# hangxu0304/DeepReduce

Measured on NVIDIA H100. Metric: ResNet-50 images/sec (whole job, device-timed, max over ranks), higher is better.
Workload: dtype bf16

## Files before the change

deepreduce_b200/ops/csrc/bn.cu:

```cuda
#include <cuda_bf16.h>

#include <algorithm>

#include "common.cuh"
#include "ops.h"

namespace dr {

namespace {

constexpr int kVec = 8;
constexpr int kApplyThreads = 256;
constexpr int kReduceThreads = 128;

struct ChanParams {
  float m[kVec], inv[kVec], w[kVec], b[kVec];
};

__device__ __forceinline__ void load8(const float* __restrict__ p, float* d) {
  const float4 a = __ldg(reinterpret_cast<const float4*>(p));
  const float4 b = __ldg(reinterpret_cast<const float4*>(p) + 1);
  d[0] = a.x; d[1] = a.y; d[2] = a.z; d[3] = a.w;
  d[4] = b.x; d[5] = b.y; d[6] = b.z; d[7] = b.w;
}

__device__ __forceinline__ void load_params(const BnParams& p, int c, ChanParams& o) {
  load8(p.mean + c, o.m);
  load8(p.invstd + c, o.inv);
  load8(p.weight + c, o.w);
  load8(p.bias + c, o.b);
}

__device__ __forceinline__ float bn_elem(float x, float m, float inv, float w, float b) {
  return __fmaf_rn(__fmul_rn(w, __fsub_rn(x, m)), inv, b);
}

__device__ __forceinline__ __nv_bfloat16 relu_bf16(__nv_bfloat16 v) {
  return __bfloat162float(v) <= 0.f ? __float2bfloat16_rn(0.f) : v;
}

__device__ __forceinline__ uint4 add_bf16x8(const uint4& a, const uint4& b) {
  uint4 s;
  const __nv_bfloat16* ha = reinterpret_cast<const __nv_bfloat16*>(&a);
  const __nv_bfloat16* hb = reinterpret_cast<const __nv_bfloat16*>(&b);
  __nv_bfloat16* hs = reinterpret_cast<__nv_bfloat16*>(&s);
#pragma unroll
  for (int i = 0; i < kVec; ++i) hs[i] = __float2bfloat16_rn(__fadd_rn(__bfloat162float(ha[i]), __bfloat162float(hb[i])));
  return s;
}

template <int kMode>
__global__ void __launch_bounds__(kApplyThreads) bn_apply_kernel(const __nv_bfloat16* __restrict__ x, BnParams px,
                                                                 const __nv_bfloat16* __restrict__ z, BnParams pz,
                                                                 __nv_bfloat16* __restrict__ out,
                                                                 uint8_t* __restrict__ mask, int64_t rows, int C) {
  const int groups = C / kVec;
  const int rows_per_cta = blockDim.x / groups;
  const int rsub = threadIdx.x / groups;
  if (rsub >= rows_per_cta) return;
  const int c = (threadIdx.x % groups) * kVec;
  ChanParams a;
  load_params(px, c, a);
  ChanParams d;
  if (kMode == 2) load_params(pz, c, d);
  const int64_t step = (int64_t)gridDim.x * rows_per_cta;
#pragma unroll 2
  for (int64_t r = (int64_t)blockIdx.x * rows_per_cta + rsub; r < rows; r += step) {
    const int64_t off = r * C + c;
    const uint4 vx = *reinterpret_cast<const uint4*>(x + off);
    uint4 vz = make_uint4(0, 0, 0, 0);
    if (kMode != 0) vz = *reinterpret_cast<const uint4*>(z + off);
    const __nv_bfloat16* hx = reinterpret_cast<const __nv_bfloat16*>(&vx);
    const __nv_bfloat16* hz = reinterpret_cast<const __nv_bfloat16*>(&vz);
    uint4 vo;
    __nv_bfloat16* ho = reinterpret_cast<__nv_bfloat16*>(&vo);
    unsigned bits = 0;
#pragma unroll
    for (int i = 0; i < kVec; ++i) {
      __nv_bfloat16 y = __float2bfloat16_rn(bn_elem(__bfloat162float(hx[i]), a.m[i], a.inv[i], a.w[i], a.b[i]));
      if (kMode != 0) {
        const __nv_bfloat16 s = kMode == 1 ? hz[i]
                                           : __float2bfloat16_rn(bn_elem(__bfloat162float(hz[i]), d.m[i], d.inv[i], d.w[i], d.b[i]));
        y = __float2bfloat16_rn(__fadd_rn(__bfloat162float(y), __bfloat162float(s)));
      }
      ho[i] = relu_bf16(y);
      bits |= (__bfloat162float(ho[i]) <= 0.f ? 0u : 1u) << i;
    }
    *reinterpret_cast<uint4*>(out + off) = vo;
    mask[r * groups + c / kVec] = (uint8_t)bits;
  }
}


__global__ void __launch_bounds__(kApplyThreads) bn_apply_pool_kernel(const __nv_bfloat16* __restrict__ x, BnParams px,
                                                                      __nv_bfloat16* __restrict__ out,
                                                                      uint8_t* __restrict__ codes, int64_t orows,
                                                                      PoolGeom pg, int C) {
  const int groups = C / kVec;
  const int rows_per_cta = blockDim.x / groups;
  const int rsub = threadIdx.x / groups;
  if (rsub >= rows_per_cta) return;
  const int c = (threadIdx.x % groups) * kVec;
  ChanParams a;
  load_params(px, c, a);
  const int64_t step = (int64_t)gridDim.x * rows_per_cta;
  for (int64_t r = (int64_t)blockIdx.x * rows_per_cta + rsub; r < orows; r += step) {
    const int ow = (int)(r % pg.Wo);
    const int64_t t = r / pg.Wo;
    const int oh = (int)(t % pg.Ho);
    const int64_t n = t / pg.Ho;
    const int h0 = 2 * oh - 1, w0 = 2 * ow - 1;
    uint4 v[9];
#pragma unroll
    for (int k = 0; k < 9; ++k) {
      const int ih = h0 + k / 3, iw = w0 + k % 3;
      v[k] = ih >= 0 && ih < pg.H && iw >= 0 && iw < pg.W
                 ? *reinterpret_cast<const uint4*>(x + ((n * pg.H + ih) * pg.W + iw) * C + c)
                 : uint4{};
    }
    __nv_bfloat16 best[kVec];
    unsigned slot[kVec];
#pragma unroll
    for (int i = 0; i < kVec; ++i) {
      best[i] = __float2bfloat16_rn(-INFINITY);
      slot[i] = 0;
    }
#pragma unroll
    for (int k = 0; k < 9; ++k) {
      const int ih = h0 + k / 3, iw = w0 + k % 3;
      if (ih < 0 || ih >= pg.H || iw < 0 || iw >= pg.W) continue;
      const __nv_bfloat16* hx = reinterpret_cast<const __nv_bfloat16*>(&v[k]);
#pragma unroll
      for (int i = 0; i < kVec; ++i) {
        const __nv_bfloat16 y = relu_bf16(__float2bfloat16_rn(bn_elem(__bfloat162float(hx[i]), a.m[i], a.inv[i], a.w[i], a.b[i])));
        const float fy = __bfloat162float(y);
        if (fy > __bfloat162float(best[i]) || isnan(fy)) {
          best[i] = y;
          slot[i] = k;
        }
      }
    }
    uint4 vo;
    __nv_bfloat16* ho = reinterpret_cast<__nv_bfloat16*>(&vo);
    uint2 vc;
    uint8_t* hc = reinterpret_cast<uint8_t*>(&vc);
#pragma unroll
    for (int i = 0; i < kVec; ++i) {
      ho[i] = best[i];
      hc[i] = (uint8_t)(slot[i] | (__bfloat162float(best[i]) <= 0.f ? 0u : 0x80u));
    }
    *reinterpret_cast<uint4*>(out + r * C + c) = vo;
    *reinterpret_cast<uint2*>(codes + r * C + c) = vc;
  }
}

struct PoolGather {
  uint4 g[4];
  uint2 code[4];
  int off;
  int nh, nw;
  int sh, sw;
};

__device__ __forceinline__ void pool_gather_codes(PoolGather& q, const uint8_t* __restrict__ codes, const PoolGeom& pg,
                                                  int row, int C, int c, bool valid) {
  const int w = row % pg.W, t = row / pg.W, h = t % pg.H, n = t / pg.H;
  const int ph = h >> 1, pw = w >> 1;
  q.nh = valid ? min((h + 1) / 2 + 1, pg.Ho) - ph : 0;
  q.nw = valid ? min((w + 1) / 2 + 1, pg.Wo) - pw : 0;
  q.sh = h - 2 * ph + 1;
  q.sw = w - 2 * pw + 1;
  q.off = ((n * pg.Ho + ph) * pg.Wo + pw) * C + c;
#pragma unroll
  for (int k = 0; k < 4; ++k) {
    const int a = k >> 1, b = k & 1;
    q.code[k] = a < q.nh && b < q.nw ? *reinterpret_cast<const uint2*>(codes + q.off + (a * pg.Wo + b) * C) : uint2{};
  }
}

template <bool kTwo>
__device__ __forceinline__ void pool_gather_grads(PoolGather& q, const __nv_bfloat16* __restrict__ gp,
                                                  const __nv_bfloat16* __restrict__ gp2, const PoolGeom& pg, int C) {
#pragma unroll
  for (int k = 0; k < 4; ++k) {
    const int a = k >> 1, b = k & 1;
    const bool in = a < q.nh && b < q.nw;
    const int off = q.off + (a * pg.Wo + b) * C;
    q.g[k] = in ? *reinterpret_cast<const uint4*>(gp + off) : uint4{};
    if (kTwo && in) q.g[k] = add_bf16x8(q.g[k], *reinterpret_cast<const uint4*>(gp2 + off));
  }
}

__device__ __forceinline__ void pool_gather_resolve(const PoolGather& q, uint4& g, unsigned& bits) {
  __nv_bfloat16* hg = reinterpret_cast<__nv_bfloat16*>(&g);
  const bool single = q.nh == 1 && q.nw == 1;
  bits = 0;
#pragma unroll
  for (int i = 0; i < kVec; ++i) {
    float s = 0.f;
    __nv_bfloat16 one = __float2bfloat16_rn(0.f);
    unsigned bit = 0;
#pragma unroll
    for (int k = 0; k < 4; ++k) {
      const int a = k >> 1, b = k & 1;
      const unsigned code = (reinterpret_cast<const uint8_t*>(&q.code[k]))[i];
      if (a < q.nh && b < q.nw && (int)(code & 0x7fu) == (q.sh - 2 * a) * 3 + (q.sw - 2 * b)) {
        const __nv_bfloat16 v = (reinterpret_cast<const __nv_bfloat16*>(&q.g[k]))[i];
        s = __fadd_rn(s, __bfloat162float(v));
        one = v;
        bit = code >> 7;
      }
    }
    hg[i] = single ? one : __float2bfloat16_rn(s);
    bits |= bit << i;
  }
}

template <bool kTwo>
__global__ void __launch_bounds__(kApplyThreads) bn_pool_grad_kernel(const __nv_bfloat16* __restrict__ gp,
                                                                     const __nv_bfloat16* __restrict__ gp2,
                                                                     const uint8_t* __restrict__ codes,
                                                                     __nv_bfloat16* __restrict__ g, PoolGeom pg,
                                                                     int64_t rows, int C) {
  const int groups = C / kVec;
  const int rows_per_cta = blockDim.x / groups;
  const int rsub = threadIdx.x / groups;
  if (rsub >= rows_per_cta) return;
  const int c = (threadIdx.x % groups) * kVec;
  const int64_t step = (int64_t)gridDim.x * rows_per_cta;
#pragma unroll 2
  for (int64_t r = (int64_t)blockIdx.x * rows_per_cta + rsub; r < rows; r += step) {
    PoolGather q;
    pool_gather_codes(q, codes, pg, (int)r, C, c, true);
    pool_gather_grads<kTwo>(q, gp, gp2, pg, C);
    uint4 v;
    unsigned bits;
    pool_gather_resolve(q, v, bits);
    __nv_bfloat16* hv = reinterpret_cast<__nv_bfloat16*>(&v);
#pragma unroll
    for (int i = 0; i < kVec; ++i)
      if (!((bits >> i) & 1u)) hv[i] = __float2bfloat16_rn(0.f);
    *reinterpret_cast<uint4*>(g + r * C + c) = v;
  }
}

struct RowTree {
  int block_y, grid_y;
  __host__ __device__ int S() const { return block_y * grid_y; }
  __host__ __device__ int loops(int rows) const { return 1 + (rows - 1) / (S() * kLoads); }
  static constexpr int kLoads = 4;
};

constexpr int kStatsThreads = 256;

__device__ __forceinline__ void welford_update(float x, float inv, float valid, float& mean, float& m2n) {
  const float d0 = __fsub_rn(x, mean);
  mean = __fmaf_rn(d0, inv, mean);
  const float d1 = __fsub_rn(x, mean);
  m2n = __fmaf_rn(__fmul_rn(d0, d1), valid, m2n);
}

template <int kN, bool kFuseNew>
__device__ __forceinline__ void welford_merge(int& n, float* mean, float* m2n, int n_new, const float* mean_new,
                                              const float* m2n_new) {
  const float fn = (float)n, fn_new = (float)n_new;
  const float factor = __frcp_rn((float)max(1, n + n_new));
#pragma unroll
  for (int i = 0; i < kN; ++i) {
    const float d = __fsub_rn(mean[i], mean_new[i]);
    const float s = kFuseNew ? __fmaf_rn(mean_new[i], fn_new, __fmul_rn(mean[i], fn))
                             : __fmaf_rn(mean[i], fn, __fmul_rn(mean_new[i], fn_new));
    mean[i] = __fmul_rn(s, factor);
    const float u = __fmul_rn(__fmul_rn(__fmul_rn(d, d), fn_new), fn);
    m2n[i] = __fadd_rn(m2n[i], __fmaf_rn(u, factor, m2n_new[i]));
  }
  n += n_new;
}

template <int kN>
struct WelfordSlots {
  float* mean; float* m2n; int* count;
  __device__ WelfordSlots(float* sh, int slots)
      : mean(sh), m2n(sh + slots * kN), count(reinterpret_cast<int*>(sh + 2 * slots * kN)) {}
  __device__ void put(int s, int n, const float* m, const float* q) const {
#pragma unroll
    for (int i = 0; i < kN; ++i) { mean[s * kN + i] = m[i]; m2n[s * kN + i] = q[i]; }
    count[s] = n;
  }
  template <bool kFuseNew>
  __device__ void merge_from(int s, int& n, float* m, float* q) const {
    float mn[kN], qn[kN];
#pragma unroll
    for (int i = 0; i < kN; ++i) { mn[i] = mean[s * kN + i]; qn[i] = m2n[s * kN + i]; }
    welford_merge<kN, kFuseNew>(n, m, q, count[s], mn, qn);
  }
  static size_t bytes(int slots) { return (size_t)slots * (2 * kN * sizeof(float) + sizeof(int)); }
};

template <int kN>
__device__ __forceinline__ void welford_tree_over_y(const WelfordSlots<kN>& sl, bool part, int y, int block_y, int base,
                                                    int stride, int& n, float* mean, float* m2n) {
  for (int off = block_y / 2; off > 0; off >>= 1) {
    if (part && y < 2 * off) sl.put(base + y * stride, n, mean, m2n);
    __syncthreads();
    if (part && y < off) sl.template merge_from<false>(base + (y + off) * stride, n, mean, m2n);
    __syncthreads();
  }
}

struct StatsOut {
  float* mean; float* invstd; float* running_mean; float* running_var;
  float* st_mean; float* st_m2n; int* st_count;
  float momentum, bessel, eps;
};

__device__ __forceinline__ void stats_store(const StatsOut& o, int c, int n, float mean, float m2n) {
  const float var = __fdiv_rn(m2n, (float)n);
  const float keep = __fsub_rn(1.f, o.momentum);
  o.mean[c] = mean;
  o.invstd[c] = rsqrtf(__fadd_rn(var, o.eps));
  o.running_mean[c] = __fmaf_rn(mean, o.momentum, __fmul_rn(o.running_mean[c], keep));
  o.running_var[c] = __fmaf_rn(__fmul_rn(var, o.bessel), o.momentum, __fmul_rn(o.running_var[c], keep));
}

__global__ void __launch_bounds__(kStatsThreads) bn_stats_kernel(const __nv_bfloat16* __restrict__ x, StatsOut o,
                                                                 RowTree t, int rows, int C) {
  constexpr int L = RowTree::kLoads;
  constexpr int kAhead = 4;
  extern __shared__ float sh[];
  const int gpc = blockDim.x / (L * t.block_y);
  const int g = threadIdx.x % gpc, j = (threadIdx.x / gpc) % L, y = threadIdx.x / (gpc * L);
  const int group = blockIdx.x * gpc + g;
  const bool live = group * kVec < C;
  const int c = live ? group * kVec : 0;
  const int S = t.S();
  const int n_loops = t.loops(rows);
  const int r0 = blockIdx.y * t.block_y + y + j * S;
  const int rstep = L * S;
  float mean[kVec], m2n[kVec];
#pragma unroll
  for (int i = 0; i < kVec; ++i) mean[i] = m2n[i] = 0.f;
  int n = 0;
  auto load = [&](uint4* b, int i0) {
#pragma unroll
    for (int u = 0; u < kAhead; ++u) {
      const int r = r0 + (i0 + u) * rstep;
      b[u] = live && i0 + u < n_loops && r < rows ? *reinterpret_cast<const uint4*>(x + (size_t)r * C + c) : uint4{};
    }
  };
  uint4 cur[kAhead];
  load(cur, 0);
  for (int i0 = 0; i0 < n_loops; i0 += kAhead) {
    uint4 nxt[kAhead];
    load(nxt, i0 + kAhead);
#pragma unroll
    for (int u = 0; u < kAhead; ++u) {
      const int i = i0 + u;
      if (i >= n_loops) break;
      const bool valid = r0 + i * rstep < rows;
      const float inv = valid ? __frcp_rn((float)(i + 1)) : 0.f;
      const float fv = valid ? 1.f : 0.f;
      n += valid;
      const __nv_bfloat16* hx = reinterpret_cast<const __nv_bfloat16*>(&cur[u]);
#pragma unroll
      for (int k = 0; k < kVec; ++k) welford_update(__bfloat162float(hx[k]), inv, fv, mean[k], m2n[k]);
    }
#pragma unroll
    for (int u = 0; u < kAhead; ++u) cur[u] = nxt[u];
  }
  const WelfordSlots<kVec> sl(sh, blockDim.x);
  sl.put(threadIdx.x, n, mean, m2n);
  __syncthreads();
  if (j == 0) {
#pragma unroll
    for (int a = 1; a < L; ++a) sl.merge_from<true>(threadIdx.x + a * gpc, n, mean, m2n);
  }
  __syncthreads();
  welford_tree_over_y<kVec>(sl, j == 0, y, t.block_y, g, gpc * L, n, mean, m2n);
  if (j != 0 || y != 0 || !live) return;
  if (t.grid_y == 1) {
#pragma unroll
    for (int i = 0; i < kVec; ++i) stats_store(o, c + i, n, mean[i], m2n[i]);
    return;
  }
#pragma unroll
  for (int i = 0; i < kVec; ++i) {
    o.st_mean[(size_t)blockIdx.y * C + c + i] = mean[i];
    o.st_m2n[(size_t)blockIdx.y * C + c + i] = m2n[i];
  }
  if (group == 0) o.st_count[blockIdx.y] = n;
}

__global__ void bn_stats_finalize_kernel(StatsOut o, RowTree t, int C) {
  extern __shared__ float sh[];
  const int cols = blockDim.x / t.block_y;
  const int col = threadIdx.x % cols, y = threadIdx.x / cols;
  const int c = blockIdx.x * cols + col;
  int n = 0;
  float mean = 0.f, m2n = 0.f;
  if (c < C)
    for (int b = y; b < t.grid_y; b += t.block_y) {
      const float mb = o.st_mean[(size_t)b * C + c], qb = o.st_m2n[(size_t)b * C + c];
      welford_merge<1, false>(n, &mean, &m2n, o.st_count[b], &mb, &qb);
    }
  const WelfordSlots<1> sl(sh, blockDim.x);
  welford_tree_over_y<1>(sl, true, y, t.block_y, col, cols, n, &mean, &m2n);
  if (y == 0 && c < C) stats_store(o, c, n, mean, m2n);
}


template <int kN>
__device__ __forceinline__ void tree_over_y(float* v, float* sh, int y, int n, int col, int width) {
  for (int off = n / 2; off > 0; off >>= 1) {
#pragma unroll
    for (int i = 0; i < kN; ++i) sh[y * width + col + i] = v[i];
    __syncthreads();
    if (y < off) {
#pragma unroll
      for (int i = 0; i < kN; ++i) v[i] = __fadd_rn(v[i], sh[(y + off) * width + col + i]);
    }
    __syncthreads();
  }
}

struct BwdOut {
  float* sums;
  float* dw; float* db; float* dwz; float* dbz;
  float* staging;
};

__device__ __forceinline__ void bwd_store(const BwdOut& o, int k, int c, int C, float v, const float* invstd,
                                         const float* invstd_z) {
  o.sums[k * C + c] = v;
  if (k == 0) {
    o.db[c] = v;
    if (o.dbz) o.dbz[c] = v;
  } else if (k == 1) {
    o.dw[c] = __fmul_rn(v, invstd[c]);
  } else {
    o.dwz[c] = __fmul_rn(v, invstd_z[c]);
  }
}

__device__ __forceinline__ float masked(__nv_bfloat16 go, unsigned bit) { return bit ? __bfloat162float(go) : 0.f; }

template <int kMode, bool kTwo>
__global__ void __launch_bounds__(kReduceThreads) bn_bwd_reduce_kernel(const __nv_bfloat16* __restrict__ go,
                                                                       const __nv_bfloat16* __restrict__ go2,
                                                                       const uint8_t* __restrict__ mask,
                                                                       const __nv_bfloat16* __restrict__ x,
                                                                       const float* __restrict__ mean,
                                                                       const float* __restrict__ invstd,
                                                                       const __nv_bfloat16* __restrict__ z,
                                                                       const float* __restrict__ mean_z,
                                                                       const float* __restrict__ invstd_z,
                                                                       __nv_bfloat16* __restrict__ g_out, BwdOut o,
                                                                       RowTree t, int rows, int C) {
  constexpr int kSums = kMode == 2 ? 3 : 2;
  constexpr int L = RowTree::kLoads;
  extern __shared__ float sh[];
  const int gpc = blockDim.x / t.block_y;
  const int tg = threadIdx.x % gpc, y = threadIdx.x / gpc;
  const int group = blockIdx.x * gpc + tg;
  const bool live = group * kVec < C;
  const int c = live ? group * kVec : 0;
  const int S = t.S();
  float m[kVec], mz[kVec];
#pragma unroll
  for (int i = 0; i < kVec; ++i) {
    m[i] = mean[c + i];
    mz[i] = kMode == 2 ? mean_z[c + i] : 0.f;
  }
  float acc[kSums][L][kVec];
#pragma unroll
  for (int k = 0; k < kSums; ++k)
#pragma unroll
    for (int j = 0; j < L; ++j)
#pragma unroll
      for (int i = 0; i < kVec; ++i) acc[k][j][i] = 0.f;
  const int mgroups = C / kVec;
  int r = blockIdx.y * t.block_y + y;
  const int n_loops = t.loops(rows);
  constexpr bool kAhead = !(kTwo && kMode == 2);
  struct Batch {
    uint4 g[L], g2[L], x[L], z[L];
    unsigned m[L];
  };
  auto load = [&](Batch& b, int r0) {
#pragma unroll
    for (int j = 0; j < L; ++j) {
      const int rr = r0 + j * S;
      if (live && rr < rows) {
        const int off = rr * C + c;
        b.g[j] = *reinterpret_cast<const uint4*>(go + off);
        if (kTwo) b.g2[j] = *reinterpret_cast<const uint4*>(go2 + off);
        b.x[j] = *reinterpret_cast<const uint4*>(x + off);
        if (kMode == 2) b.z[j] = *reinterpret_cast<const uint4*>(z + off);
        b.m[j] = kMode == 3 ? 0u : mask[rr * mgroups + group];
      } else {
        b.g[j] = uint4{}; b.g2[j] = uint4{}; b.x[j] = uint4{}; b.z[j] = uint4{}; b.m[j] = 0;
      }
    }
  };
  Batch cur;
  if (kAhead) load(cur, r);
  for (int it = 0; it < n_loops; ++it) {
    if (!kAhead) load(cur, r);
    if (kTwo) {
#pragma unroll
      for (int j = 0; j < L; ++j) cur.g[j] = add_bf16x8(cur.g[j], cur.g2[j]);
    }
    Batch nxt;
    if (kAhead) load(nxt, r + L * S);
    const unsigned* mb = cur.m;
#pragma unroll
    for (int j = 0; j < L; ++j) {
      const __nv_bfloat16* hg = reinterpret_cast<const __nv_bfloat16*>(&cur.g[j]);
      const __nv_bfloat16* hx = reinterpret_cast<const __nv_bfloat16*>(&cur.x[j]);
      const __nv_bfloat16* hz = reinterpret_cast<const __nv_bfloat16*>(&cur.z[j]);
      uint4 vo;
      __nv_bfloat16* ho = reinterpret_cast<__nv_bfloat16*>(&vo);
#pragma unroll
      for (int i = 0; i < kVec; ++i) {
        const unsigned bit = (mb[j] >> i) & 1u;
        const float g = kMode == 3 ? __bfloat162float(hg[i]) : masked(hg[i], bit);
        if (kMode == 1) ho[i] = bit ? hg[i] : __float2bfloat16_rn(0.f);
        acc[0][j][i] = __fadd_rn(acc[0][j][i], g);
        acc[1][j][i] = __fmaf_rn(__fsub_rn(__bfloat162float(hx[i]), m[i]), g, acc[1][j][i]);
        if (kMode == 2) acc[2][j][i] = __fmaf_rn(__fsub_rn(__bfloat162float(hz[i]), mz[i]), g, acc[2][j][i]);
      }
      if (kMode == 1 && live && r + j * S < rows) *reinterpret_cast<uint4*>(g_out + (r + j * S) * C + c) = vo;
    }
    if (kAhead) cur = nxt;
    r += L * S;
  }
#pragma unroll
  for (int k = 0; k < kSums; ++k) {
#pragma unroll
    for (int i = 0; i < kVec; ++i)
#pragma unroll
      for (int j = 1; j < L; ++j) acc[k][0][i] = __fadd_rn(acc[k][0][i], acc[k][j][i]);
    tree_over_y<kVec>(acc[k][0], sh, y, t.block_y, tg * kVec, gpc * kVec);
  }
  if (y != 0 || !live) return;
#pragma unroll
  for (int k = 0; k < kSums; ++k)
#pragma unroll
    for (int i = 0; i < kVec; ++i) {
      if (t.grid_y > 1) o.staging[((size_t)k * t.grid_y + blockIdx.y) * C + c + i] = acc[k][0][i];
      else bwd_store(o, k, c + i, C, acc[k][0][i], invstd, invstd_z);
    }
}

__global__ void bn_bwd_finalize_kernel(BwdOut o, RowTree t, int n_sums, int C, const float* __restrict__ invstd,
                                       const float* __restrict__ invstd_z) {
  extern __shared__ float sh[];
  const int cols = blockDim.x / t.block_y;
  const int col = threadIdx.x % cols, y = threadIdx.x / cols;
  const int c = blockIdx.x * cols + col;
  for (int k = 0; k < n_sums; ++k) {
    float v = 0.f;
    if (c < C)
      for (int b = y; b < t.grid_y; b += t.block_y) v = __fadd_rn(v, o.staging[((size_t)k * t.grid_y + b) * C + c]);
    tree_over_y<1>(&v, sh, y, t.block_y, col, cols);
    if (y == 0 && c < C) bwd_store(o, k, c, C, v, invstd, invstd_z);
  }
}

struct ElemtChan {
  float m[kVec], f1[kVec], f2[kVec], sdy[kVec];
};

__device__ __forceinline__ void elemt_params(const float* mean, const float* invstd, const float* w, const float* sdy,
                                             const float* sxmu, float norm, int c, ElemtChan& p) {
  float inv[kVec], ww[kVec], sx[kVec];
  load8(mean + c, p.m);
  load8(invstd + c, inv);
  load8(w + c, ww);
  load8(sdy + c, p.sdy);
  load8(sxmu + c, sx);
#pragma unroll
  for (int i = 0; i < kVec; ++i) {
    p.f1[i] = __fmul_rn(__fmul_rn(__fmul_rn(inv[i], inv[i]), sx[i]), norm);
    p.f2[i] = __fmul_rn(ww[i], inv[i]);
  }
}

__device__ __forceinline__ __nv_bfloat16 elemt(float g, float x, const ElemtChan& p, int i, float norm) {
  const float a = __fmaf_rn(-p.sdy[i], norm, g);
  return __float2bfloat16_rn(__fmul_rn(__fmaf_rn(-p.f1[i], __fsub_rn(x, p.m[i]), a), p.f2[i]));
}

struct ElemtArgs {
  const float *mean, *invstd, *weight, *sums;
  const float *mean_z, *invstd_z, *weight_z;
};

template <int kMode, bool kTwo>
__global__ void __launch_bounds__(kApplyThreads) bn_bwd_elemt_kernel(const __nv_bfloat16* __restrict__ g_in,
                                                                     const __nv_bfloat16* __restrict__ g2_in,
                                                                     const uint8_t* __restrict__ mask,
                                                                     const __nv_bfloat16* __restrict__ x,
                                                                     const __nv_bfloat16* __restrict__ z, ElemtArgs a,
                                                                     __nv_bfloat16* __restrict__ dx,
                                                                     __nv_bfloat16* __restrict__ dz, float norm,
                                                                     int64_t rows, int C) {
  const int groups = C / kVec;
  const int rows_per_cta = blockDim.x / groups;
  const int rsub = threadIdx.x / groups;
  if (rsub >= rows_per_cta) return;
  const int c = (threadIdx.x % groups) * kVec;
  ElemtChan p;
  elemt_params(a.mean, a.invstd, a.weight, a.sums, a.sums + C, norm, c, p);
  ElemtChan q;
  if (kMode == 2) elemt_params(a.mean_z, a.invstd_z, a.weight_z, a.sums, a.sums + 2 * C, norm, c, q);
  const int64_t step = (int64_t)gridDim.x * rows_per_cta;
#pragma unroll 2
  for (int64_t r = (int64_t)blockIdx.x * rows_per_cta + rsub; r < rows; r += step) {
    const int64_t off = r * C + c;
    uint4 vg = *reinterpret_cast<const uint4*>(g_in + off);
    if (kTwo) vg = add_bf16x8(vg, *reinterpret_cast<const uint4*>(g2_in + off));
    const unsigned mb = kMode == 1 || kMode == 3 ? 0xffu : mask[r * groups + c / kVec];
    const uint4 vx = *reinterpret_cast<const uint4*>(x + off);
    uint4 vz = make_uint4(0, 0, 0, 0);
    if (kMode == 2) vz = *reinterpret_cast<const uint4*>(z + off);
    const __nv_bfloat16* hg = reinterpret_cast<const __nv_bfloat16*>(&vg);
    const __nv_bfloat16* hx = reinterpret_cast<const __nv_bfloat16*>(&vx);
    const __nv_bfloat16* hz = reinterpret_cast<const __nv_bfloat16*>(&vz);
    uint4 vo, vd;
    __nv_bfloat16* ho = reinterpret_cast<__nv_bfloat16*>(&vo);
    __nv_bfloat16* hd = reinterpret_cast<__nv_bfloat16*>(&vd);
#pragma unroll
    for (int i = 0; i < kVec; ++i) {
      const float g = masked(hg[i], (mb >> i) & 1u);
      ho[i] = elemt(g, __bfloat162float(hx[i]), p, i, norm);
      if (kMode == 2) hd[i] = elemt(g, __bfloat162float(hz[i]), q, i, norm);
    }
    *reinterpret_cast<uint4*>(dx + off) = vo;
    if (kMode == 2) *reinterpret_cast<uint4*>(dz + off) = vd;
  }
}

__global__ void bn_update_stats_kernel(const float* __restrict__ mean, float* __restrict__ var_invstd,
                                       float* __restrict__ running_mean, float* __restrict__ running_var, int C,
                                       float momentum, float bessel, float eps) {
  const int c = blockIdx.x * blockDim.x + threadIdx.x;
  if (c >= C) return;
  const float m = mean[c], v = var_invstd[c];
  const float unbiased_var = v * bessel;
  running_mean[c] = m * momentum + (1 - momentum) * running_mean[c];
  running_var[c] = unbiased_var * momentum + (1 - momentum) * running_var[c];
  var_invstd[c] = rsqrtf(v + eps);
}

template <typename K>
cudaError_t rows_grid(K kernel, int64_t rows, int C, int& grid, int& threads) {
  const int groups = C / kVec;
  const int rows_per_cta = groups >= kApplyThreads ? 1 : kApplyThreads / groups;
  threads = groups * rows_per_cta;
  int per_sm = 0;
  cudaError_t e = cudaOccupancyMaxActiveBlocksPerMultiprocessor(&per_sm, kernel, threads, 0);
  if (e != cudaSuccess) return e;
  int64_t g = (rows + rows_per_cta - 1) / rows_per_cta;
  const int64_t cap = (int64_t)(per_sm > 0 ? per_sm : 1) * sm_count();
  grid = (int)(g > cap ? cap : g);
  return cudaSuccess;
}

template <int kMode>
cudaError_t launch_apply(const void* x, const BnParams& px, const void* z, const BnParams& pz, void* out, void* mask,
                         int64_t rows, int C, cudaStream_t st) {
  if (rows == 0) return cudaSuccess;
  int grid = 0, threads = 0;
  cudaError_t e = rows_grid(bn_apply_kernel<kMode>, rows, C, grid, threads);
  if (e != cudaSuccess) return e;
  count_launch();
  bn_apply_kernel<kMode><<<grid, threads, 0, st>>>(reinterpret_cast<const __nv_bfloat16*>(x), px,
                                                   reinterpret_cast<const __nv_bfloat16*>(z), pz,
                                                   reinterpret_cast<__nv_bfloat16*>(out),
                                                   reinterpret_cast<uint8_t*>(mask), rows, C);
  return cudaGetLastError();
}

int last_pow2(unsigned n) {
  n |= n >> 1; n |= n >> 2; n |= n >> 4; n |= n >> 8; n |= n >> 16;
  return std::max<int>(1, (int)(n - (n >> 1)));
}

RowTree row_tree(int rows, int C) {
  const int block_x = std::min(last_pow2((unsigned)C), 32);
  const int block_y = std::min(last_pow2((unsigned)((rows + 15) / 16)), 512 / block_x);
  int grid_y = std::min((rows + block_y * 16 - 1) / (block_y * 16), 128);
  if (grid_y < 8) grid_y = 1;
  return {block_y, grid_y};
}

template <int kMode, bool kTwo>
cudaError_t launch_bwd_reduce(const BnBwd& b, const RowTree& t, const BwdOut& o, int rows, int C, cudaStream_t st) {
  const int groups = C / kVec;
  const int gpc = std::min(groups, std::max(1, kReduceThreads / t.block_y));
  const dim3 grid((groups + gpc - 1) / gpc, t.grid_y);
  const int threads = gpc * t.block_y;
  count_launch();
  bn_bwd_reduce_kernel<kMode, kTwo><<<grid, threads, threads * kVec * sizeof(float), st>>>(
      reinterpret_cast<const __nv_bfloat16*>(b.go), reinterpret_cast<const __nv_bfloat16*>(b.go2), b.mask,
      reinterpret_cast<const __nv_bfloat16*>(b.x), b.px.mean, b.px.invstd, reinterpret_cast<const __nv_bfloat16*>(b.z),
      b.pz.mean, b.pz.invstd, reinterpret_cast<__nv_bfloat16*>(b.g), o, t, rows, C);
  return cudaGetLastError();
}

template <int kMode, bool kTwo>
cudaError_t launch_bwd_elemt(const BnBwd& b, const ElemtArgs& a, int64_t rows, int C, cudaStream_t st) {
  int grid = 0, threads = 0;
  cudaError_t e = rows_grid(bn_bwd_elemt_kernel<kMode, kTwo>, rows, C, grid, threads);
  if (e != cudaSuccess) return e;
  const float norm = (float)(1.0 / (double)rows);
  count_launch();
  bn_bwd_elemt_kernel<kMode, kTwo><<<grid, threads, 0, st>>>(
      reinterpret_cast<const __nv_bfloat16*>(kMode == 1 || kMode == 3 ? b.g : b.go),
      reinterpret_cast<const __nv_bfloat16*>(b.go2), b.mask, reinterpret_cast<const __nv_bfloat16*>(b.x),
      reinterpret_cast<const __nv_bfloat16*>(b.z), a, reinterpret_cast<__nv_bfloat16*>(b.dx),
      reinterpret_cast<__nv_bfloat16*>(b.dz), norm, rows, C);
  return cudaGetLastError();
}

template <int kMode, bool kTwo>
cudaError_t launch_backward(const BnBwd& b, int64_t rows64, int C, cudaStream_t st) {
  const int rows = (int)rows64;
  const RowTree t = row_tree(rows, C);
  const BwdOut o{b.sums, b.dw, b.db, b.dwz, b.dbz, b.staging};
  cudaError_t e;
  if (kMode == 3) {
    int grid = 0, threads = 0;
    e = rows_grid(bn_pool_grad_kernel<kTwo>, rows64, C, grid, threads);
    if (e != cudaSuccess) return e;
    count_launch();
    bn_pool_grad_kernel<kTwo><<<grid, threads, 0, st>>>(reinterpret_cast<const __nv_bfloat16*>(b.go),
                                                        reinterpret_cast<const __nv_bfloat16*>(b.go2), b.mask,
                                                        reinterpret_cast<__nv_bfloat16*>(b.g), b.pool, rows64, C);
    e = cudaGetLastError();
    if (e != cudaSuccess) return e;
  }
  BnBwd bb = b;
  if (kMode == 3) bb.go = b.g;
  e = launch_bwd_reduce<kMode, kTwo && kMode != 3>(bb, t, o, rows, C, st);
  if (e != cudaSuccess) return e;
  if (t.grid_y > 1) {
    const int cols = std::max(1, 512 / t.block_y);
    const int threads = cols * t.block_y;
    count_launch();
    bn_bwd_finalize_kernel<<<(C + cols - 1) / cols, threads, threads * sizeof(float), st>>>(
        o, t, kMode == 2 ? 3 : 2, C, b.px.invstd, b.pz.invstd);
    e = cudaGetLastError();
    if (e != cudaSuccess) return e;
  }
  const ElemtArgs a{b.px.mean, b.px.invstd, b.px.weight, b.sums, b.pz.mean, b.pz.invstd, b.pz.weight};
  return launch_bwd_elemt<kMode, kTwo && kMode == 2>(b, a, rows64, C, st);
}

cudaError_t launch_stats(const BnStats& s, int rows, int C, cudaStream_t st) {
  const RowTree t = row_tree(rows, C);
  const int grid_y = t.grid_y;
  const StatsOut o{s.mean, s.invstd, s.running_mean, s.running_var,
                   s.staging, s.staging + (size_t)grid_y * C, reinterpret_cast<int*>(s.staging + 2 * (size_t)grid_y * C),
                   s.momentum, s.bessel, s.eps};
  const int groups = C / kVec;
  const int gpc = std::min(groups, std::max(1, kStatsThreads / (RowTree::kLoads * t.block_y)));
  const int threads = gpc * RowTree::kLoads * t.block_y;
  count_launch();
  bn_stats_kernel<<<dim3((groups + gpc - 1) / gpc, grid_y), threads, WelfordSlots<kVec>::bytes(threads), st>>>(
      reinterpret_cast<const __nv_bfloat16*>(s.x), o, t, rows, C);
  cudaError_t e = cudaGetLastError();
  if (e != cudaSuccess || grid_y == 1) return e;
  const int cols = std::max(1, 512 / t.block_y);
  const int fthreads = cols * t.block_y;
  count_launch();
  bn_stats_finalize_kernel<<<(C + cols - 1) / cols, fthreads, WelfordSlots<1>::bytes(fthreads), st>>>(o, t, C);
  return cudaGetLastError();
}

}

void bn_row_tree(int64_t rows, int C, int* block_y, int* grid_y) {
  const RowTree t = row_tree((int)rows, C);
  *block_y = t.block_y;
  *grid_y = t.grid_y;
}

cudaError_t launch_bn_backward(int mode, const BnBwd& b, int64_t rows, int C, cudaStream_t st) {
  if (rows == 0) return cudaSuccess;
  const bool two = b.go2 != nullptr;
  switch (mode) {
    case 0: return two ? cudaErrorInvalidValue : launch_backward<0, false>(b, rows, C, st);
    case 1: return two ? launch_backward<1, true>(b, rows, C, st) : launch_backward<1, false>(b, rows, C, st);
    case 2: return two ? launch_backward<2, true>(b, rows, C, st) : launch_backward<2, false>(b, rows, C, st);
    case 3: return two ? launch_backward<3, true>(b, rows, C, st) : launch_backward<3, false>(b, rows, C, st);
    default: return cudaErrorInvalidValue;
  }
}

cudaError_t launch_bn_stats(const BnStats& s, int64_t rows, int C, cudaStream_t st) {
  if (rows == 0) return cudaSuccess;
  return launch_stats(s, (int)rows, C, st);
}

cudaError_t launch_bn_update_stats(const float* mean, float* var_invstd, float* running_mean, float* running_var, int C,
                                   float momentum, float bessel, float eps, cudaStream_t st) {
  count_launch();
  bn_update_stats_kernel<<<(C + 255) / 256, 256, 0, st>>>(mean, var_invstd, running_mean, running_var, C, momentum,
                                                          bessel, eps);
  return cudaGetLastError();
}

cudaError_t launch_bn_apply(int mode, const void* x, const BnParams& px, const void* z, const BnParams& pz, void* out,
                            void* mask, int64_t rows, int C, cudaStream_t st) {
  switch (mode) {
    case 0: return launch_apply<0>(x, px, z, pz, out, mask, rows, C, st);
    case 1: return launch_apply<1>(x, px, z, pz, out, mask, rows, C, st);
    case 2: return launch_apply<2>(x, px, z, pz, out, mask, rows, C, st);
    default: return cudaErrorInvalidValue;
  }
}

cudaError_t launch_bn_apply_pool(const void* x, const BnParams& px, void* out, void* codes, int N, const PoolGeom& pg,
                                 int C, cudaStream_t st) {
  const int64_t orows = (int64_t)N * pg.Ho * pg.Wo;
  if (orows == 0) return cudaSuccess;
  int grid = 0, threads = 0;
  cudaError_t e = rows_grid(bn_apply_pool_kernel, orows, C, grid, threads);
  if (e != cudaSuccess) return e;
  count_launch();
  bn_apply_pool_kernel<<<grid, threads, 0, st>>>(reinterpret_cast<const __nv_bfloat16*>(x), px,
                                                 reinterpret_cast<__nv_bfloat16*>(out),
                                                 reinterpret_cast<uint8_t*>(codes), orows, pg, C);
  return cudaGetLastError();
}

}
```

deepreduce_b200/ops/csrc/common.cuh:

```cuda
#pragma once
#include <cuda_runtime.h>
#include <stdint.h>

#include "plan.h"

#define DR_HD __host__ __device__ __forceinline__
#define DR_D __device__ __forceinline__

namespace dr {

constexpr uint32_t kGolden = 0x9E3779B1u;
constexpr uint32_t kBAdd = 0x7F4A7C15u;
constexpr int kThreads = 512;
constexpr int kPerThread = kTile / kThreads;
constexpr int kWarps = kThreads / 32;

DR_HD uint32_t fmix32(uint32_t h) {
  h ^= h >> 16; h *= 0x85EBCA6Bu; h ^= h >> 13; h *= 0xC2B2AE35u; h ^= h >> 16;
  return h;
}

struct HashAB { uint32_t a, b; };

DR_HD HashAB hash_ab(uint32_t x, uint32_t seed) {
  uint32_t y = x ^ seed;
  HashAB r;
  r.a = fmix32(y);
  r.b = fmix32(y * kGolden + kBAdd) | 1u;
  return r;
}

DR_HD uint32_t mulhi32(uint32_t h, uint32_t m) {
#ifdef __CUDA_ARCH__
  return __umulhi(h, m);
#else
  return (uint32_t)(((uint64_t)h * (uint64_t)m) >> 32);
#endif
}

DR_HD uint32_t policy_hash(uint32_t x, uint32_t seed) {
  return fmix32((x * kGolden + seed) ^ 0x5BD1E995u);
}

DR_HD uint32_t policy_seed(uint32_t step, uint32_t tensor_id) {
  return fmix32((step * 0x01000193u) ^ ((tensor_id + 1u) * kGolden));
}

template <typename LoadFn>
DR_D bool bloom_test(uint32_t x, uint32_t seed, uint32_t n_hash, uint32_t m_bits, LoadFn ld) {
  HashAB h = hash_ab(x, seed);
  uint32_t v = h.a;
  uint32_t j = 0;
  for (; j + 1 < n_hash; j += 2) {
    const uint32_t p0 = mulhi32(v, m_bits), p1 = mulhi32(v + h.b, m_bits);
    const uint32_t w0 = ld(p0 >> 5), w1 = ld(p1 >> 5);
    if (!((w0 >> (p0 & 31u)) & (w1 >> (p1 & 31u)) & 1u)) return false;
    v += 2u * h.b;
  }
  if (j < n_hash) {
    const uint32_t p0 = mulhi32(v, m_bits);
    if (!((ld(p0 >> 5) >> (p0 & 31u)) & 1u)) return false;
  }
  return true;
}

DR_D void bloom_set(uint32_t* filter, uint32_t x, uint32_t seed, uint32_t n_hash, uint32_t m_bits) {
  HashAB h = hash_ab(x, seed);
  uint32_t v = h.a;
  for (uint32_t j = 0; j < n_hash; ++j) {
    uint32_t pos = mulhi32(v, m_bits);
    atomicOr(filter + (pos >> 5), 1u << (pos & 31u));
    v += h.b;
  }
}

DR_D uint32_t ld_acquire_gpu(const uint32_t* p) {
  uint32_t v; asm volatile("ld.acquire.gpu.global.u32 %0, [%1];" : "=r"(v) : "l"(p) : "memory"); return v;
}
DR_D uint64_t ld_acquire_gpu64(const uint64_t* p) {
  uint64_t v; asm volatile("ld.acquire.gpu.global.u64 %0, [%1];" : "=l"(v) : "l"(p) : "memory"); return v;
}
DR_D void st_release_gpu64(uint64_t* p, uint64_t v) {
  asm volatile("st.release.gpu.global.u64 [%0], %1;" :: "l"(p), "l"(v) : "memory");
}
DR_D uint32_t ld_acquire_sys(const uint32_t* p) {
  uint32_t v; asm volatile("ld.acquire.sys.global.u32 %0, [%1];" : "=r"(v) : "l"(p) : "memory"); return v;
}
DR_D void st_release_sys(uint32_t* p, uint32_t v) {
  asm volatile("st.release.sys.global.u32 [%0], %1;" :: "l"(p), "r"(v) : "memory");
}
DR_D uint32_t ld_relaxed_sys(const uint32_t* p) {
  uint32_t v; asm volatile("ld.relaxed.sys.global.u32 %0, [%1];" : "=r"(v) : "l"(p) : "memory"); return v;
}
DR_D float4 ld_stream_f4(const float4* p) {
  float4 r;
  asm volatile("ld.global.L1::no_allocate.v4.f32 {%0,%1,%2,%3}, [%4];"
               : "=f"(r.x), "=f"(r.y), "=f"(r.z), "=f"(r.w) : "l"(p));
  return r;
}
DR_D uint4 ld_stream_u4(const uint4* p) {
  uint4 r;
  asm volatile("ld.global.L1::no_allocate.v4.u32 {%0,%1,%2,%3}, [%4];"
               : "=r"(r.x), "=r"(r.y), "=r"(r.z), "=r"(r.w) : "l"(p));
  return r;
}

DR_D uint32_t smem_u32(const void* p) { return (uint32_t)__cvta_generic_to_shared(p); }
DR_D void mbar_init(uint64_t* bar, uint32_t count) {
  asm volatile("mbarrier.init.shared::cta.b64 [%0], %1;" :: "r"(smem_u32(bar)), "r"(count) : "memory");
}
DR_D void mbar_inval(uint64_t* bar) {
  asm volatile("mbarrier.inval.shared::cta.b64 [%0];" :: "r"(smem_u32(bar)) : "memory");
}
DR_D void mbar_fence_init() { asm volatile("fence.mbarrier_init.release.cluster;" ::: "memory"); }
DR_D void fence_proxy_async() { asm volatile("fence.proxy.async;" ::: "memory"); }
DR_D void fence_proxy_async_smem() { asm volatile("fence.proxy.async.shared::cta;" ::: "memory"); }
DR_D void mbar_expect_tx(uint64_t* bar, uint32_t bytes) {
  asm volatile("mbarrier.arrive.expect_tx.shared::cta.b64 _, [%0], %1;" :: "r"(smem_u32(bar)), "r"(bytes) : "memory");
}
DR_D void bulk_g2s(void* dst_smem, const void* src_gmem, uint32_t bytes, uint64_t* bar) {
  asm volatile("cp.async.bulk.shared::cluster.global.mbarrier::complete_tx::bytes [%0], [%1], %2, [%3];"
               :: "r"(smem_u32(dst_smem)), "l"(src_gmem), "r"(bytes), "r"(smem_u32(bar)) : "memory");
}
DR_D void mbar_arrive(uint64_t* bar) {
  asm volatile("mbarrier.arrive.shared::cta.b64 _, [%0];" :: "r"(smem_u32(bar)) : "memory");
}
DR_D uint64_t globaltimer_ns() {
  uint64_t t; asm volatile("mov.u64 %0, %%globaltimer;" : "=l"(t)); return t;
}
DR_D void mbar_wait(uint64_t* bar, uint32_t parity, uint32_t* status = nullptr) {
  uint32_t ok, spins = 0;
  do {
    if (++spins > (1u << 24)) { if (status) atomicExch(status, 5u); break; }
    asm volatile("{\n\t.reg .pred p;\n\tmbarrier.try_wait.parity.shared::cta.b64 p, [%1], %2;\n\tselp.u32 %0, 1, 0, p;\n\t}"
                 : "=r"(ok) : "r"(smem_u32(bar)), "r"(parity) : "memory");
  } while (!ok);
}

DR_D void cp_async_8(void* dst_smem, const void* src_gmem) {
  asm volatile("cp.async.ca.shared.global [%0], [%1], 8;" :: "r"(smem_u32(dst_smem)), "l"(src_gmem) : "memory");
}
DR_D void cp_async_4(void* dst_smem, const void* src_gmem) {
  asm volatile("cp.async.ca.shared.global [%0], [%1], 4;" :: "r"(smem_u32(dst_smem)), "l"(src_gmem) : "memory");
}
DR_D void cp_async_16(void* dst_smem, const void* src_gmem) {
  asm volatile("cp.async.cg.shared.global [%0], [%1], 16;" :: "r"(smem_u32(dst_smem)), "l"(src_gmem) : "memory");
}
DR_D void cp_async_commit() { asm volatile("cp.async.commit_group;" ::: "memory"); }
template <int N>
DR_D void cp_async_wait() { asm volatile("cp.async.wait_group %0;" :: "n"(N) : "memory"); }

DR_D void multimem_st_v4(uint4* mc_addr, uint4 v) {
  asm volatile("multimem.st.weak.global.v4.f32 [%0], {%1,%2,%3,%4};"
               :: "l"(mc_addr), "f"(__uint_as_float(v.x)), "f"(__uint_as_float(v.y)), "f"(__uint_as_float(v.z)),
                  "f"(__uint_as_float(v.w)) : "memory");
}

DR_D void multimem_st_v2(uint2* mc_addr, uint2 v) {
  asm volatile("multimem.st.weak.global.v2.f32 [%0], {%1,%2};"
               :: "l"(mc_addr), "f"(__uint_as_float(v.x)), "f"(__uint_as_float(v.y)) : "memory");
}
DR_D void multimem_st_b32(uint32_t* mc_addr, uint32_t v) {
  asm volatile("multimem.st.weak.global.f32 [%0], %1;" :: "l"(mc_addr), "f"(__uint_as_float(v)) : "memory");
}

DR_D void grid_barrier(uint32_t* counter, uint32_t& epoch, uint32_t* status, uint32_t spin_limit) {
  fence_proxy_async();
  __syncthreads();
  if (threadIdx.x == 0) {
    epoch += 1;
    const uint32_t target = epoch * gridDim.x;
    __threadfence();
    atomicAdd(counter, 1u);
    uint32_t spins = 0;
    while (ld_acquire_gpu(counter) < target) {
      __nanosleep(32);
      if (++spins > spin_limit) { atomicExch(status, 4u); break; }
    }
    __threadfence();
  }
  __syncthreads();
}

template <int kDegP1>
DR_D void gram_eval(float x, float N, int deg_eff, float (&p)[kDegP1]) {
  p[0] = 1.f;
#pragma unroll
  for (int k = 1; k < kDegP1; ++k) p[k] = 0.f;
  if (deg_eff >= 1) {
    const float u = N - 2.f * x;
    p[1] = u / N;
#pragma unroll
    for (int k = 1; k < kDegP1 - 1; ++k) {
      if (k < deg_eff)
        p[k + 1] = ((2.f * k + 1.f) * u * p[k] - (float)k * (N + k + 1.f) * p[k - 1]) / ((k + 1.f) * (N - k));
    }
  }
}

void count_launch(int n = 1);
long long launch_count();

int sm_count();

}
```

Baseline: 6091.

## Pipeline BN backward reduce with cp.async ring and persistent grid

Rewrites the BN backward reduce kernel as a persistent grid that walks work items and prefetches input batches into a multi-stage shared-memory ring with zero-fill cp.async. The goal is to keep more loads in flight and hide memory latency. The stats and bwd finalize kernels now batch their partial-sum loads, and occupancy queries are cached on the host. In exchange the kernel uses more shared memory, which can lower occupancy, and the persistent loop adds more index arithmetic.

```diff
diff --git a/deepreduce_b200/ops/csrc/bn.cu b/deepreduce_b200/ops/csrc/bn.cu
--- a/deepreduce_b200/ops/csrc/bn.cu
+++ b/deepreduce_b200/ops/csrc/bn.cu
@@ -1,6 +1,8 @@
 #include <cuda_bf16.h>
 
 #include <algorithm>
+#include <mutex>
+#include <vector>
 
 #include "common.cuh"
 #include "ops.h"
@@ -391,7 +393,10 @@
   if (group == 0) o.st_count[blockIdx.y] = n;
 }
 
+constexpr int kFinalizeBatch = 8;
+
 __global__ void bn_stats_finalize_kernel(StatsOut o, RowTree t, int C) {
+  constexpr int B = kFinalizeBatch;
   extern __shared__ float sh[];
   const int cols = blockDim.x / t.block_y;
   const int col = threadIdx.x % cols, y = threadIdx.x / cols;
@@ -399,9 +404,20 @@
   int n = 0;
   float mean = 0.f, m2n = 0.f;
   if (c < C)
-    for (int b = y; b < t.grid_y; b += t.block_y) {
-      const float mb = o.st_mean[(size_t)b * C + c], qb = o.st_m2n[(size_t)b * C + c];
-      welford_merge<1, false>(n, &mean, &m2n, o.st_count[b], &mb, &qb);
+    for (int b0 = y; b0 < t.grid_y; b0 += B * t.block_y) {
+      float mb[B], qb[B];
+      int nb[B];
+#pragma unroll
+      for (int u = 0; u < B; ++u) {
+        const int b = b0 + u * t.block_y;
+        const bool in = b < t.grid_y;
+        mb[u] = in ? o.st_mean[(size_t)b * C + c] : 0.f;
+        qb[u] = in ? o.st_m2n[(size_t)b * C + c] : 0.f;
+        nb[u] = in ? o.st_count[b] : 0;
+      }
+#pragma unroll
+      for (int u = 0; u < B; ++u)
+        if (b0 + u * t.block_y < t.grid_y) welford_merge<1, false>(n, &mean, &m2n, nb[u], &mb[u], &qb[u]);
     }
   const WelfordSlots<1> sl(sh, blockDim.x);
   welford_tree_over_y<1>(sl, true, y, t.block_y, col, cols, n, &mean, &m2n);
@@ -443,6 +459,16 @@
 }
 
 __device__ __forceinline__ float masked(__nv_bfloat16 go, unsigned bit) { return bit ? __bfloat162float(go) : 0.f; }
+
+template <int kMode, bool kTwo>
+struct ReduceRing {
+  static constexpr int kVecs = 2 + (kTwo ? 1 : 0) + (kMode == 2 ? 1 : 0);
+  static constexpr bool kMask = kMode != 3;
+  static constexpr int kBatchBytes = RowTree::kLoads * (16 * kVecs + (kMask ? 4 : 0));
+  static constexpr int kAheadBytes = 512;
+  static constexpr int kDepth = 1 + (kAheadBytes + kBatchBytes - 1) / kBatchBytes;
+  static size_t bytes(int threads) { return (size_t)threads * (kDepth * kBatchBytes + kVec * sizeof(float)); }
+};
 
 template <int kMode, bool kTwo>
 __global__ void __launch_bounds__(kReduceThreads) bn_bwd_reduce_kernel(const __nv_bfloat16* __restrict__ go,
@@ -455,115 +481,165 @@
                                                                        const float* __restrict__ mean_z,
                                                                        const float* __restrict__ invstd_z,
                                                                        __nv_bfloat16* __restrict__ g_out, BwdOut o,
-                                                                       RowTree t, int rows, int C) {
+                                                                       RowTree t, int rows, int C, int grid_x) {
+  using Ring = ReduceRing<kMode, kTwo>;
   constexpr int kSums = kMode == 2 ? 3 : 2;
   constexpr int L = RowTree::kLoads;
-  extern __shared__ float sh[];
-  const int gpc = blockDim.x / t.block_y;
+  constexpr int D = Ring::kDepth, V = Ring::kVecs;
+  extern __shared__ uint4 ring_sh[];
+  const int nt = blockDim.x;
+  uint4* vring = ring_sh;
+  uint32_t* mring = reinterpret_cast<uint32_t*>(ring_sh + D * L * V * nt);
+  float* sh = reinterpret_cast<float*>(mring + (Ring::kMask ? D * L * nt : 0));
+  const int gpc = nt / t.block_y;
   const int tg = threadIdx.x % gpc, y = threadIdx.x / gpc;
-  const int group = blockIdx.x * gpc + tg;
-  const bool live = group * kVec < C;
-  const int c = live ? group * kVec : 0;
   const int S = t.S();
+  const int n_loops = t.loops(rows);
+  const int mgroups = C / kVec;
+  const int items = grid_x * t.grid_y;
+  const int n_batches = (items - blockIdx.x + gridDim.x - 1) / gridDim.x * n_loops;
+
+  int pk = 0, pit = 0, ps = 0, pq = 0;
+  auto issue = [&]() {
+    if (pq < n_batches) {
+      const int item = blockIdx.x + pk * gridDim.x;
+      const int group = (item % grid_x) * gpc + tg;
+      const bool live = group * kVec < C;
+      const int r0 = (item / grid_x) * t.block_y + y + pit * L * S;
+#pragma unroll
+      for (int j = 0; j < L; ++j) {
+        const int rr = r0 + j * S;
+        const bool ok = live && rr < rows;
+        const int off = ok ? rr * C + group * kVec : 0;
+        const uint32_t n = ok ? 16u : 0u;
+        uint4* slot = vring + ((ps * L + j) * V) * nt + threadIdx.x;
+        int v = 0;
+        cp_async_16_zfill(slot + (v++) * nt, go + off, n);
+        if (kTwo) cp_async_16_zfill(slot + (v++) * nt, go2 + off, n);
+        cp_async_16_zfill(slot + (v++) * nt, x + off, n);
+        if (kMode == 2) cp_async_16_zfill(slot + (v++) * nt, z + off, n);
+        if (Ring::kMask) {
+          const int moff = ok ? rr * mgroups + group : 0;
+          cp_async_4_zfill(mring + (ps * L + j) * nt + threadIdx.x, mask + (moff & ~3), ok ? 4u : 0u);
+        }
+      }
+      if (++pit == n_loops) { pit = 0; ++pk; }
+      if (++ps == D) ps = 0;
+      ++pq;
+    }
+    cp_async_commit();
+  };
+#pragma unroll 1
+  for (int d = 0; d < D - 1; ++d) issue();
+
+  int group = 0, c = 0, by = 0, it = 0, k_item = 0, cs = 0;
+  bool live = false;
   float m[kVec], mz[kVec];
-#pragma unroll
-  for (int i = 0; i < kVec; ++i) {
-    m[i] = mean[c + i];
-    mz[i] = kMode == 2 ? mean_z[c + i] : 0.f;
-  }
   float acc[kSums][L][kVec];
-#pragma unroll
-  for (int k = 0; k < kSums; ++k)
-#pragma unroll
-    for (int j = 0; j < L; ++j)
-#pragma unroll
-      for (int i = 0; i < kVec; ++i) acc[k][j][i] = 0.f;
-  const int mgroups = C / kVec;
-  int r = blockIdx.y * t.block_y + y;
-  const int n_loops = t.loops(rows);
-  constexpr bool kAhead = !(kTwo && kMode == 2);
-  struct Batch {
-    uint4 g[L], g2[L], x[L], z[L];
-    unsigned m[L];
+  auto begin_item = [&]() {
+    const int item = blockIdx.x + k_item * gridDim.x;
+    group = (item % grid_x) * gpc + tg;
+    by = item / grid_x;
+    live = group * kVec < C;
+    c = live ? group * kVec : 0;
+#pragma unroll
+    for (int i = 0; i < kVec; ++i) {
+      m[i] = mean[c + i];
+      mz[i] = kMode == 2 ? mean_z[c + i] : 0.f;
+    }
+#pragma unroll
+    for (int k = 0; k < kSums; ++k)
+#pragma unroll
+      for (int j = 0; j < L; ++j)
+#pragma unroll
+        for (int i = 0; i < kVec; ++i) acc[k][j][i] = 0.f;
   };
-  auto load = [&](Batch& b, int r0) {
+  begin_item();
+#pragma unroll 1
+  for (int q = 0; q < n_batches; ++q) {
+    issue();
+    cp_async_wait<D - 1>();
+    const int r = by * t.block_y + y + it * L * S;
 #pragma unroll
     for (int j = 0; j < L; ++j) {
-      const int rr = r0 + j * S;
-      if (live && rr < rows) {
-        const int off = rr * C + c;
-        b.g[j] = *reinterpret_cast<const uint4*>(go + off);
-        if (kTwo) b.g2[j] = *reinterpret_cast<const uint4*>(go2 + off);
-        b.x[j] = *reinterpret_cast<const uint4*>(x + off);
-        if (kMode == 2) b.z[j] = *reinterpret_cast<const uint4*>(z + off);
-        b.m[j] = kMode == 3 ? 0u : mask[rr * mgroups + group];
-      } else {
-        b.g[j] = uint4{}; b.g2[j] = uint4{}; b.x[j] = uint4{}; b.z[j] = uint4{}; b.m[j] = 0;
-      }
-    }
-  };
-  Batch cur;
-  if (kAhead) load(cur, r);
-  for (int it = 0; it < n_loops; ++it) {
-    if (!kAhead) load(cur, r);
-    if (kTwo) {
-#pragma unroll
-      for (int j = 0; j < L; ++j) cur.g[j] = add_bf16x8(cur.g[j], cur.g2[j]);
-    }
-    Batch nxt;
-    if (kAhead) load(nxt, r + L * S);
-    const unsigned* mb = cur.m;
-#pragma unroll
-    for (int j = 0; j < L; ++j) {
-      const __nv_bfloat16* hg = reinterpret_cast<const __nv_bfloat16*>(&cur.g[j]);
-      const __nv_bfloat16* hx = reinterpret_cast<const __nv_bfloat16*>(&cur.x[j]);
-      const __nv_bfloat16* hz = reinterpret_cast<const __nv_bfloat16*>(&cur.z[j]);
+      const uint4* slot = vring + ((cs * L + j) * V) * nt + threadIdx.x;
+      uint4 vg = slot[0];
+      if (kTwo) vg = add_bf16x8(vg, slot[nt]);
+      const uint4 vx = slot[(kTwo ? 2 : 1) * nt];
+      const uint4 vz = kMode == 2 ? slot[(kTwo ? 3 : 2) * nt] : uint4{};
+      const int rr = r + j * S;
+      const unsigned mb = Ring::kMask ? mring[(cs * L + j) * nt + threadIdx.x] >> (8 * ((rr * mgroups + group) & 3)) : 0u;
+      const __nv_bfloat16* hg = reinterpret_cast<const __nv_bfloat16*>(&vg);
+      const __nv_bfloat16* hx = reinterpret_cast<const __nv_bfloat16*>(&vx);
+      const __nv_bfloat16* hz = reinterpret_cast<const __nv_bfloat16*>(&vz);
       uint4 vo;
       __nv_bfloat16* ho = reinterpret_cast<__nv_bfloat16*>(&vo);
 #pragma unroll
       for (int i = 0; i < kVec; ++i) {
-        const unsigned bit = (mb[j] >> i) & 1u;
+        const unsigned bit = (mb >> i) & 1u;
         const float g = kMode == 3 ? __bfloat162float(hg[i]) : masked(hg[i], bit);
         if (kMode == 1) ho[i] = bit ? hg[i] : __float2bfloat16_rn(0.f);
         acc[0][j][i] = __fadd_rn(acc[0][j][i], g);
         acc[1][j][i] = __fmaf_rn(__fsub_rn(__bfloat162float(hx[i]), m[i]), g, acc[1][j][i]);
         if (kMode == 2) acc[2][j][i] = __fmaf_rn(__fsub_rn(__bfloat162float(hz[i]), mz[i]), g, acc[2][j][i]);
       }
-      if (kMode == 1 && live && r + j * S < rows) *reinterpret_cast<uint4*>(g_out + (r + j * S) * C + c) = vo;
-    }
-    if (kAhead) cur = nxt;
-    r += L * S;
-  }
-#pragma unroll
-  for (int k = 0; k < kSums; ++k) {
-#pragma unroll
-    for (int i = 0; i < kVec; ++i)
-#pragma unroll
-      for (int j = 1; j < L; ++j) acc[k][0][i] = __fadd_rn(acc[k][0][i], acc[k][j][i]);
-    tree_over_y<kVec>(acc[k][0], sh, y, t.block_y, tg * kVec, gpc * kVec);
-  }
-  if (y != 0 || !live) return;
-#pragma unroll
-  for (int k = 0; k < kSums; ++k)
-#pragma unroll
-    for (int i = 0; i < kVec; ++i) {
-      if (t.grid_y > 1) o.staging[((size_t)k * t.grid_y + blockIdx.y) * C + c + i] = acc[k][0][i];
-      else bwd_store(o, k, c + i, C, acc[k][0][i], invstd, invstd_z);
-    }
+      if (kMode == 1 && live && rr < rows) *reinterpret_cast<uint4*>(g_out + rr * C + c) = vo;
+    }
+    if (++cs == D) cs = 0;
+    if (++it < n_loops) continue;
+#pragma unroll
+    for (int k = 0; k < kSums; ++k) {
+#pragma unroll
+      for (int i = 0; i < kVec; ++i)
+#pragma unroll
+        for (int j = 1; j < L; ++j) acc[k][0][i] = __fadd_rn(acc[k][0][i], acc[k][j][i]);
+      tree_over_y<kVec>(acc[k][0], sh, y, t.block_y, tg * kVec, gpc * kVec);
+    }
+    if (y == 0 && live) {
+#pragma unroll
+      for (int k = 0; k < kSums; ++k)
+#pragma unroll
+        for (int i = 0; i < kVec; ++i) {
+          if (t.grid_y > 1) o.staging[((size_t)k * t.grid_y + by) * C + c + i] = acc[k][0][i];
+          else bwd_store(o, k, c + i, C, acc[k][0][i], invstd, invstd_z);
+        }
+    }
+    it = 0;
+    ++k_item;
+    if (q + 1 < n_batches) begin_item();
+  }
+  cp_async_wait<0>();
 }
 
 __global__ void bn_bwd_finalize_kernel(BwdOut o, RowTree t, int n_sums, int C, const float* __restrict__ invstd,
                                        const float* __restrict__ invstd_z) {
+  constexpr int B = kFinalizeBatch, kMaxSums = 3;
   extern __shared__ float sh[];
   const int cols = blockDim.x / t.block_y;
   const int col = threadIdx.x % cols, y = threadIdx.x / cols;
   const int c = blockIdx.x * cols + col;
-  for (int k = 0; k < n_sums; ++k) {
-    float v = 0.f;
-    if (c < C)
-      for (int b = y; b < t.grid_y; b += t.block_y) v = __fadd_rn(v, o.staging[((size_t)k * t.grid_y + b) * C + c]);
-    tree_over_y<1>(&v, sh, y, t.block_y, col, cols);
-    if (y == 0 && c < C) bwd_store(o, k, c, C, v, invstd, invstd_z);
+  float v[kMaxSums] = {0.f, 0.f, 0.f};
+  if (c < C)
+    for (int b0 = y; b0 < t.grid_y; b0 += B * t.block_y) {
+      float s[kMaxSums][B];
+#pragma unroll
+      for (int k = 0; k < kMaxSums; ++k)
+#pragma unroll
+        for (int u = 0; u < B; ++u) {
+          const int b = b0 + u * t.block_y;
+          s[k][u] = k < n_sums && b < t.grid_y ? o.staging[((size_t)k * t.grid_y + b) * C + c] : 0.f;
+        }
+#pragma unroll
+      for (int k = 0; k < kMaxSums; ++k)
+#pragma unroll
+        for (int u = 0; u < B; ++u)
+          if (b0 + u * t.block_y < t.grid_y) v[k] = __fadd_rn(v[k], s[k][u]);
+    }
+#pragma unroll
+  for (int k = 0; k < kMaxSums; ++k) {
+    if (k >= n_sums) break;
+    tree_over_y<1>(&v[k], sh, y, t.block_y, col, cols);
+    if (y == 0 && c < C) bwd_store(o, k, c, C, v[k], invstd, invstd_z);
   }
 }
 
@@ -653,16 +729,40 @@
   var_invstd[c] = rsqrtf(v + eps);
 }
 
+cudaError_t blocks_per_sm(const void* kernel, int threads, size_t smem, int max_smem, int& per_sm) {
+  struct Entry { int dev; const void* kernel; int threads; size_t smem; int per_sm; };
+  static std::mutex mu;
+  static std::vector<Entry> cache;
+  int dev = 0;
+  cudaError_t e = cudaGetDevice(&dev);
+  if (e != cudaSuccess) return e;
+  std::lock_guard<std::mutex> lock(mu);
+  for (const Entry& c : cache)
+    if (c.dev == dev && c.kernel == kernel && c.threads == threads && c.smem == smem) {
+      per_sm = c.per_sm;
+      return cudaSuccess;
+    }
+  if (max_smem > 0) {
+    e = cudaFuncSetAttribute(kernel, cudaFuncAttributeMaxDynamicSharedMemorySize, max_smem);
+    if (e != cudaSuccess) return e;
+  }
+  e = cudaOccupancyMaxActiveBlocksPerMultiprocessor(&per_sm, kernel, threads, smem);
+  if (e != cudaSuccess) return e;
+  per_sm = std::max(per_sm, 1);
+  cache.push_back({dev, kernel, threads, smem, per_sm});
+  return cudaSuccess;
+}
+
 template <typename K>
 cudaError_t rows_grid(K kernel, int64_t rows, int C, int& grid, int& threads) {
   const int groups = C / kVec;
   const int rows_per_cta = groups >= kApplyThreads ? 1 : kApplyThreads / groups;
   threads = groups * rows_per_cta;
   int per_sm = 0;
-  cudaError_t e = cudaOccupancyMaxActiveBlocksPerMultiprocessor(&per_sm, kernel, threads, 0);
+  cudaError_t e = blocks_per_sm(reinterpret_cast<const void*>(kernel), threads, 0, 0, per_sm);
   if (e != cudaSuccess) return e;
   int64_t g = (rows + rows_per_cta - 1) / rows_per_cta;
-  const int64_t cap = (int64_t)(per_sm > 0 ? per_sm : 1) * sm_count();
+  const int64_t cap = (int64_t)per_sm * sm_count();
   grid = (int)(g > cap ? cap : g);
   return cudaSuccess;
 }
@@ -697,15 +797,24 @@
 
 template <int kMode, bool kTwo>
 cudaError_t launch_bwd_reduce(const BnBwd& b, const RowTree& t, const BwdOut& o, int rows, int C, cudaStream_t st) {
+  using Ring = ReduceRing<kMode, kTwo>;
+  if (Ring::kMask && reinterpret_cast<uintptr_t>(b.mask) % 4 != 0) return cudaErrorMisalignedAddress;
   const int groups = C / kVec;
   const int gpc = std::min(groups, std::max(1, kReduceThreads / t.block_y));
-  const dim3 grid((groups + gpc - 1) / gpc, t.grid_y);
+  const int grid_x = (groups + gpc - 1) / gpc;
   const int threads = gpc * t.block_y;
+  const size_t smem = Ring::bytes(threads);
+  auto kernel = bn_bwd_reduce_kernel<kMode, kTwo>;
+  int per_sm = 0;
+  cudaError_t e = blocks_per_sm(reinterpret_cast<const void*>(kernel), threads, smem, (int)Ring::bytes(kReduceThreads),
+                                per_sm);
+  if (e != cudaSuccess) return e;
+  const int grid = (int)std::min<int64_t>((int64_t)grid_x * t.grid_y, (int64_t)per_sm * sm_count());
   count_launch();
-  bn_bwd_reduce_kernel<kMode, kTwo><<<grid, threads, threads * kVec * sizeof(float), st>>>(
+  kernel<<<grid, threads, smem, st>>>(
       reinterpret_cast<const __nv_bfloat16*>(b.go), reinterpret_cast<const __nv_bfloat16*>(b.go2), b.mask,
       reinterpret_cast<const __nv_bfloat16*>(b.x), b.px.mean, b.px.invstd, reinterpret_cast<const __nv_bfloat16*>(b.z),
-      b.pz.mean, b.pz.invstd, reinterpret_cast<__nv_bfloat16*>(b.g), o, t, rows, C);
+      b.pz.mean, b.pz.invstd, reinterpret_cast<__nv_bfloat16*>(b.g), o, t, rows, C, grid_x);
   return cudaGetLastError();
 }
 
diff --git a/deepreduce_b200/ops/csrc/common.cuh b/deepreduce_b200/ops/csrc/common.cuh
--- a/deepreduce_b200/ops/csrc/common.cuh
+++ b/deepreduce_b200/ops/csrc/common.cuh
@@ -145,6 +145,14 @@
 }
 DR_D void cp_async_16(void* dst_smem, const void* src_gmem) {
   asm volatile("cp.async.cg.shared.global [%0], [%1], 16;" :: "r"(smem_u32(dst_smem)), "l"(src_gmem) : "memory");
+}
+DR_D void cp_async_16_zfill(void* dst_smem, const void* src_gmem, uint32_t src_size) {
+  asm volatile("cp.async.cg.shared.global [%0], [%1], 16, %2;" :: "r"(smem_u32(dst_smem)), "l"(src_gmem), "r"(src_size)
+               : "memory");
+}
+DR_D void cp_async_4_zfill(void* dst_smem, const void* src_gmem, uint32_t src_size) {
+  asm volatile("cp.async.ca.shared.global [%0], [%1], 4, %2;" :: "r"(smem_u32(dst_smem)), "l"(src_gmem), "r"(src_size)
+               : "memory");
 }
 DR_D void cp_async_commit() { asm volatile("cp.async.commit_group;" ::: "memory"); }
 template <int N>
```

Measured after the change: 6137 (median of 6 runs). About the same (+0.7%).
